# CityU-AIM-Group/SCAN

Hardware: AMD Instinct MI355X
Metric: train images/sec (whole node), VGG16 C2F 1024x2048 (higher is better)
Workload: dtype f32 (fp32 storage, fp32 multiply, fp32 accumulate -- the reference's arithmetic; the convolutions run it on the bf16 matrix cores as bf16x6: every fp32 operand cut into 3 bf16 pieces = all 24 significand bits, 6 bf16 MFMAs per product)

## Files before the change

### include/scan_hip.h

```cpp
#ifndef SCAN_HIP_H
#define SCAN_HIP_H

#include <stdint.h>

#ifdef __cplusplus
extern "C" {
#endif

#define SCAN_MAX_LEVELS 5

typedef struct {
  int32_t n_levels;
  int32_t n_images;
  int32_t h[SCAN_MAX_LEVELS];
  int32_t w[SCAN_MAX_LEVELS];
  int64_t row_off[SCAN_MAX_LEVELS + 1];
} scan_pyramid_t;

const char* scan_last_error(void);
int scan_abi_version(void);

#define SCAN_TUNE_UNKNOWN (-2147483647 - 1)
int scan_tune(const char* key, int value);
int scan_tune_get(const char* key);
// ... 377 lines not shown
int scan_gconv3x3_to1_dgrad(const float* dy, int32_t Ns, const scan_pyramid_t* d, int32_t G, int32_t Cg, const float* w,
                            const float* mask, float* dx, void* stream);
int scan_gconv3x3_to1_wgrad(const float* x, const float* dy, int32_t Ns, const scan_pyramid_t* d, int32_t G, int32_t Cg,
                            float* dw, int32_t accumulate, float* ws, void* stream);
int scan_gconv3x3_to1_backward(const float* x, const float* dy, int32_t Ns, const scan_pyramid_t* d, int32_t G, int32_t Cg,
                               const float* w, int32_t relu_mask, float* dx, float* dw, int32_t accumulate, float* ws,
                               void* stream);
int32_t scan_gconv3x3_to1_max_groups(void);
#define SCAN_GCONV_RUNS 1
#define SCAN_GCONV_LANE_MAPPED 2
#define SCAN_GCONV_BITS 4
#define SCAN_GCONV_ACT 8
int32_t scan_gconv3x3_to1_caps(int32_t G, int32_t Cg);
int scan_gconv3x3_to1_any_forward(const float* x, const scan_pyramid_t* d, int32_t G, int32_t Cg, const float* w,
                                  const float* bias, float* y, int32_t Ns, float* ws, void* stream);
int scan_gconv3x3_to1_any_dgrad(const float* dy, int32_t Ns, const scan_pyramid_t* d, int32_t G, int32_t Cg, const float* w,
                                const float* mask, float* dx, void* stream);
int scan_gconv3x3_to1_any_wgrad(const float* x, const float* dy, int32_t Ns, const scan_pyramid_t* d, int32_t G, int32_t Cg,
                                float* dw, int32_t accumulate, float* ws, void* stream);
int scan_gconv3x3_to1_any_backward(const float* x, const float* dy, int32_t Ns, const scan_pyramid_t* d, int32_t G, int32_t Cg,
                                   const float* w, int32_t relu_mask, float* dx, float* dw, int32_t accumulate, float* ws,
                                   void* stream);
int64_t scan_gconv3x3_to1_act_ws_floats(const scan_pyramid_t* d, int32_t G, int32_t Cg);
int scan_gconv3x3_to1_act_forward(const float* x, const scan_pyramid_t* d, int32_t G, int32_t Cg, const float* w,
                                  const float* bias, const float* a, int32_t lda, int32_t a_col0, const float* E, float* y,
                                  int32_t Ns, float* ws, void* stream);
int scan_gconv3x3_to1_act_backward(const float* x, const float* dy, int32_t Ns, const scan_pyramid_t* d, int32_t G, int32_t Cg,
                                   const float* w, const float* a, int32_t lda, int32_t a_col0, const float* E, float* dx,
                                   float* dw, int32_t accumulate, float* ws, void* stream);
int scan_gconv3x3_to1_act_grads(const float* dh, const scan_pyramid_t* d, int32_t G, int32_t Cg, const float* a, int32_t lda,
                                int32_t a_col0, const float* E, float* da, int32_t ldda, int32_t da_col0, float* dE,
                                int32_t accumulate, float* ws, void* stream);
int scan_gconv3x3_to1_act_backward_all(const float* x, const float* dy, int32_t Ns, const scan_pyramid_t* d, int32_t G,
                                       int32_t Cg, const float* w, const float* a, int32_t lda, int32_t a_col0, const float* E,
                                       float* dx, float* dw, float* da, int32_t ldda, int32_t da_col0, float* dE,
                                       int32_t accumulate, float* ws, void* stream);
int scan_gconv3x3_to1_forward_bits(const float* x, const scan_pyramid_t* d, int32_t G, int32_t Cg, const float* w,
                                   const float* bias, float* y, int32_t Ns, float* ws, uint32_t* relu_bits, void* stream);
int scan_gconv3x3_to1_backward_bits(const float* x, const float* dy, int32_t Ns, const scan_pyramid_t* d, int32_t G,
                                    int32_t Cg, const float* w, const uint32_t* relu_bits, float* dx, float* dw,
                                    int32_t accumulate, float* ws, void* stream);

int scan_resize_bilinear_u8(const uint8_t* src, int32_t H, int32_t W, uint8_t* tmp, uint8_t* dst, int32_t OH, int32_t OW,
                            const int32_t* xbounds, const int32_t* xcoef, int32_t kx, const int32_t* ybounds,
                            const int32_t* ycoef, int32_t ky, void* stream);

// ... 59 lines not shown
```

### scan_amd/_lib.py

```python
import ctypes
import os

_HERE = os.path.dirname(os.path.abspath(__file__))
LIB_PATH = os.environ.get("SCAN_HIP_LIB") or os.path.join(_HERE, "libscan_hip.so")

MAX_LEVELS = 5
TUNE_UNKNOWN = -2 ** 31
NMS_PANEL = 8192
NMS_MAX = 262144

c_i32, c_i64, c_f32, c_vp = ctypes.c_int32, ctypes.c_int64, ctypes.c_float, ctypes.c_void_p


class PyramidDesc(ctypes.Structure):
    _fields_ = [("n_levels", c_i32), ("n_images", c_i32), ("h", c_i32 * MAX_LEVELS), ("w", c_i32 * MAX_LEVELS),
                ("row_off", c_i64 * (MAX_LEVELS + 1))]


_PD = ctypes.POINTER(PyramidDesc)


class SgdSegment(ctypes.Structure):
    _fields_ = [("p", c_vp), ("g", c_vp), ("buf", c_vp), ("n", c_i64), ("lr", c_f32), ("wd", c_f32),
                ("first_step", c_i32), ("reserved", c_i32)]
# ... 178 lines not shown
    "scan_cka_unstack_grads": (ctypes.c_int, [ctypes.POINTER(CkaBranch), c_i32, c_i32, c_i32, c_i64, c_i64, c_i64, c_i64,
                                              c_i64, c_i32, c_i32, c_vp, c_vp, c_vp, c_vp, c_i32, c_vp]),
    "scan_gconv3x3_to1_ws_floats": (c_i64, [_PD, c_i32, c_i32]),
    "scan_gconv3x3_to1_max_groups": (c_i32, []),
    "scan_gconv3x3_to1_caps": (c_i32, [c_i32, c_i32]),
    "scan_gconv3x3_to1_any_forward": (ctypes.c_int, [c_vp, _PD, c_i32, c_i32, c_vp, c_vp, c_vp, c_i32, c_vp, c_vp]),
    "scan_gconv3x3_to1_any_dgrad": (ctypes.c_int, [c_vp, c_i32, _PD, c_i32, c_i32, c_vp, c_vp, c_vp, c_vp]),
    "scan_gconv3x3_to1_any_wgrad": (ctypes.c_int, [c_vp, c_vp, c_i32, _PD, c_i32, c_i32, c_vp, c_i32, c_vp, c_vp]),
    "scan_gconv3x3_to1_any_backward": (ctypes.c_int, [c_vp, c_vp, c_i32, _PD, c_i32, c_i32, c_vp, c_i32, c_vp, c_vp, c_i32,
                                                      c_vp, c_vp]),
    "scan_gconv3x3_to1_forward": (ctypes.c_int, [c_vp, _PD, c_i32, c_i32, c_vp, c_vp, c_vp, c_i32, c_vp, c_vp]),
    "scan_gconv3x3_to1_dgrad": (ctypes.c_int, [c_vp, c_i32, _PD, c_i32, c_i32, c_vp, c_vp, c_vp, c_vp]),
    "scan_gconv3x3_to1_wgrad": (ctypes.c_int, [c_vp, c_vp, c_i32, _PD, c_i32, c_i32, c_vp, c_i32, c_vp, c_vp]),
    "scan_gconv3x3_to1_backward": (ctypes.c_int, [c_vp, c_vp, c_i32, _PD, c_i32, c_i32, c_vp, c_i32, c_vp, c_vp, c_i32, c_vp,
                                                  c_vp]),
    "scan_gconv3x3_to1_forward_bits": (ctypes.c_int, [c_vp, _PD, c_i32, c_i32, c_vp, c_vp, c_vp, c_i32, c_vp, c_vp, c_vp]),
    "scan_gconv3x3_to1_backward_bits": (ctypes.c_int, [c_vp, c_vp, c_i32, _PD, c_i32, c_i32, c_vp, c_vp, c_vp, c_vp, c_i32,
                                                       c_vp, c_vp]),
    "scan_cka_stack_weights_split": (ctypes.c_int, [ctypes.POINTER(CkaBranch), c_i32, c_i32, c_i32, c_i64, c_i64, c_i64, c_i64,
                                                    c_i64, c_i32, c_vp, c_vp, c_vp, c_vp, c_vp, c_vp]),
    "scan_cka_unstack_grads_split": (ctypes.c_int, [ctypes.POINTER(CkaBranch), c_i32, c_i32, c_i32, c_i64, c_i64, c_i64, c_i64,
                                                    c_i64, c_i32, c_vp, c_vp, c_vp, c_vp, c_vp, c_i32, c_vp]),
    "scan_gconv3x3_to1_act_ws_floats": (c_i64, [_PD, c_i32, c_i32]),
    "scan_gconv3x3_to1_act_forward": (ctypes.c_int, [c_vp, _PD, c_i32, c_i32, c_vp, c_vp, c_vp, c_i32, c_i32, c_vp, c_vp, c_i32,
                                                     c_vp, c_vp]),
    "scan_gconv3x3_to1_act_backward": (ctypes.c_int, [c_vp, c_vp, c_i32, _PD, c_i32, c_i32, c_vp, c_vp, c_i32, c_i32, c_vp, c_vp,
                                                      c_vp, c_i32, c_vp, c_vp]),
    "scan_gconv3x3_to1_act_backward_all": (ctypes.c_int, [c_vp, c_vp, c_i32, _PD, c_i32, c_i32, c_vp, c_vp, c_i32, c_i32, c_vp,
                                                          c_vp, c_vp, c_vp, c_i32, c_i32, c_vp, c_i32, c_vp, c_vp]),
    "scan_gconv3x3_to1_act_grads": (ctypes.c_int, [c_vp, _PD, c_i32, c_i32, c_vp, c_i32, c_i32, c_vp, c_vp, c_i32, c_i32, c_vp,
                                                   c_i32, c_vp, c_vp]),
    "scan_resize_bilinear_u8": (ctypes.c_int, [c_vp, c_i32, c_i32, c_vp, c_vp, c_i32, c_i32, c_vp, c_vp, c_i32, c_vp, c_vp,
                                               c_i32, c_vp]),
    "scan_sigmoid_focal_loss_ordered_ws_floats": (c_i64, [c_i64, c_i32]),
    "scan_sigmoid_focal_loss_forward_ordered": (ctypes.c_int, [c_vp, c_vp, c_i64, c_i32, c_f32, c_f32, c_vp, c_vp, c_vp, c_vp]),
    "scan_iou_loss_ordered_ws_floats": (c_i64, [c_i64]),
    "scan_iou_loss_forward_ordered": (ctypes.c_int, [c_vp, c_vp, c_vp, c_i64, c_vp, c_vp, c_vp]),
    "scan_bce_logits_ordered_ws_floats": (c_i64, [c_i64]),
    "scan_bce_logits_forward_ordered": (ctypes.c_int, [c_vp, c_vp, c_f32, c_vp, c_i64, c_i64, c_vp, c_vp, c_vp]),
    "scan_cka_bce_ordered_ws_floats": (c_i64, [c_i64, c_i32]),
    "scan_cka_bce_forward_ordered": (ctypes.c_int, [c_vp, c_vp, c_i64, c_i32, c_f32, c_vp, c_vp, c_vp]),
    "scan_cka_bce_forward_loss_ordered": (ctypes.c_int, [c_vp, c_vp, c_i64, c_i32, c_f32, c_vp, c_vp, c_vp]),
    "scan_softmax_focal_ordered_ws_floats": (c_i64, [c_i64]),
    "scan_softmax_focal_forward_ordered": (ctypes.c_int, [c_vp, c_vp, c_i64, c_i32, c_f32, c_vp, c_vp, c_vp]),
    "scan_groupnorm_ordered_ws_floats": (c_i64, [_PD, c_i32, c_i32]),
    "scan_groupnorm_stats_ordered": (ctypes.c_int, [c_vp, _PD, c_i32, c_i32, c_f32, c_vp, c_vp, c_vp]),
# ... 85 lines not shown
```

### scan_amd/csrc/capi.cpp

```cpp
#include <stdarg.h>
#include <stdio.h>
#include <string.h>

#include "../../include/scan_hip.h"
#include "conv_launch.h"

static thread_local char g_err[512] = "";

extern "C" void scan_set_error(const char* fmt, ...) {
  va_list ap;
  va_start(ap, fmt);
  vsnprintf(g_err, sizeof(g_err), fmt, ap);
  va_end(ap);
}

extern "C" const char* scan_last_error(void) { return g_err; }
extern "C" int scan_abi_version(void) { return 1; }

int g_scan_deterministic = 0;

struct Knob {
  const char* key;
  int* slot;
  int dflt;
};
static Knob* knob_table(int* count) {
  static Knob knobs[] = {
      {"conv_bn256", &g_scan_conv_bn256, 0},   {"conv_v2", &g_scan_conv_v2, 0},         {"conv_wg1024", &g_scan_conv_wg1024, 0},
      {"conv_w8", &g_scan_conv_w8, 0},         {"conv_tpb3", &g_scan_conv_tpb3, 0},     {"conv_bn64_th16", &g_scan_conv_bn64_th16, 0},
      {"conv_glds", &g_scan_conv_glds, 0},     {"wgrad_v6", &g_scan_wgrad_v6, 0},       {"wgrad_prio", &g_scan_wgrad_prio, 0},
      {"wgrad_tile", &g_scan_wgrad_tile, 0},   {"wgrad_wgs", &g_scan_wgrad_wgs, 0},     {"gconv_mfma", &g_scan_gconv_mfma, 0},
      {"dbscan_bf16x3", &g_scan_dbscan_bf16x3, 0}, {"reduce_blocks", &g_scan_reduce_blocks, 0}, {"conv1x1", &g_scan_conv1x1, 0},
      {"conv_wino", &g_scan_conv_wino, 0},     {"wgrad_wino", &g_scan_wgrad_wino, 0},   {"wino_tpb", &g_scan_wino_tpb, 0},
      {"deterministic", &g_scan_deterministic, 0}, {"dynconv_generic", &g_scan_dynconv_generic, 0},
  };
  static bool init = false;
  if (!init) {
    for (auto& k : knobs) k.dflt = *k.slot;
    init = true;
  }
  *count = (int)(sizeof(knobs) / sizeof(knobs[0]));
  return knobs;
}
static Knob* find_knob(const char* key) {
  int n = 0;
  Knob* t = knob_table(&n);
  if (key == nullptr) return nullptr;
  for (int i = 0; i < n; ++i)
    if (strcmp(key, t[i].key) == 0) return &t[i];
  return nullptr;
}

extern "C" int scan_tune(const char* key, int value) {
  Knob* k = find_knob(key);
  if (k == nullptr) return SCAN_TUNE_UNKNOWN;
  const int old = *k->slot;
  *k->slot = value;
// ... 19 lines not shown
```

### scan_amd/csrc/conv_launch.h

```cpp
#pragma once
#include <hip/hip_runtime_api.h>
#include <stdint.h>

#include "../../include/scan_hip.h"

extern int g_scan_conv_v2;
extern int g_scan_conv_bn256, g_scan_conv_wg1024, g_scan_conv_w8, g_scan_conv_tpb3;
extern int g_scan_conv_glds, g_scan_conv_bn64_th16, g_scan_conv1x1;
extern int g_scan_conv_wino, g_scan_wino_tpb;
extern int g_scan_wgrad_v6, g_scan_wgrad_prio, g_scan_wgrad_tile, g_scan_wgrad_wgs, g_scan_wgrad_wino;
extern int g_scan_gconv_mfma;
extern int g_scan_dynconv_generic;
extern int g_scan_dbscan_bf16x3;
extern int g_scan_reduce_blocks;

struct ConvArgs {
  const float* x;
  const scan_pyramid_t* od;
  const scan_pyramid_t* sd;
  int32_t Cs;
  const __bf16* w[3];
  int32_t Csw;
  const float* bias;
  const float* mask;
  float* y;
  int32_t Nout, Ns, relu, map;
  hipStream_t st;
  double* gn_ws;
};

struct ConvInst {
  int id;
  void (*launch)(const ConvArgs&);
};
// ... 17 lines not shown
```

### scan_amd/csrc/gconv.hip

```cpp
#include "common.h"

#define GC_G 128

template <int CTRL, int ROW_MASK>
__device__ __forceinline__ float dpp_add(float v) {
  const int r = __builtin_amdgcn_update_dpp(0, __builtin_bit_cast(int, v), CTRL, ROW_MASK, 0xF, false);
  return v + __builtin_bit_cast(float, r);
}
__device__ __forceinline__ float half_wave_sum_hi(float v) {
  v = dpp_add<0xB1, 0xF>(v);
  v = dpp_add<0x4E, 0xF>(v);
  v = dpp_add<0x141, 0xF>(v);
  v = dpp_add<0x140, 0xF>(v);
  v = dpp_add<0x142, 0xA>(v);
  return v;
}

__device__ __forceinline__ int64_t neighbour_row(const scan_pyramid_t& d, int64_t m, const RowCoord& rc, int oy, int ox) {
  const int y = rc.y + oy, x = rc.x + ox;
  if (y < 0 || y >= d.h[rc.lvl] || x < 0 || x >= d.w[rc.lvl]) return -1;
  return m + (int64_t)oy * d.w[rc.lvl] + ox;
}

__device__ __forceinline__ float4 zero4() { return make_float4(0.f, 0.f, 0.f, 0.f); }
// ... 34 lines not shown
template <int SIGN>
__device__ __forceinline__ void tap_values(const scan_pyramid_t& d, int64_t q, const RowCoord& rc,
                                           const float* __restrict__ src, int ld, int g, bool uniform, float (&v)[9]) {
  if (uniform) {
    const int g0 = 2 * (int)(threadIdx.x >> 6);
    const int l = threadIdx.x & 63;
    const int tl = l % 9, gl = l / 9;
    const int64_t pl = l < 18 ? neighbour_row(d, q, rc, SIGN * (tl / 3 - 1), SIGN * (tl % 3 - 1)) : -1;
    const float val = pl >= 0 ? src[pl * ld + g0 + gl] : 0.f;
    const int vb = __builtin_bit_cast(int, val);
    const bool hi = (l & 32) != 0;
#pragma unroll
    for (int t = 0; t < 9; ++t) {
      const float lo_v = __builtin_bit_cast(float, __builtin_amdgcn_readlane(vb, t));
      const float hi_v = __builtin_bit_cast(float, __builtin_amdgcn_readlane(vb, 9 + t));
      v[t] = hi ? hi_v : lo_v;
    }
  } else {
#pragma unroll
    for (int t = 0; t < 9; ++t) {
      const int64_t p = neighbour_row(d, q, rc, SIGN * (t / 3 - 1), SIGN * (t % 3 - 1));
      v[t] = p >= 0 ? src[p * ld + g] : 0.f;
    }
  }
}

struct LaneMap {
  int g, l32, coff;
  int64_t first, stride, step;
  bool uniform;
};

__device__ __forceinline__ LaneMap slot_lanes(int GC, int un, bool runs) {
  const int quads = GC >> 2;
  const int slots = 256 / quads;
  const int cq = threadIdx.x % quads, slot = threadIdx.x / quads;
  LaneMap lm;
  lm.g = cq >> 5, lm.l32 = cq & 31, lm.coff = 4 * cq;
  lm.first = runs ? (int64_t)blockIdx.x * un * slots + slot : (int64_t)blockIdx.x * slots + slot;
  lm.stride = runs ? (int64_t)slots : (int64_t)gridDim.x * slots;
  lm.step = (int64_t)gridDim.x * un * slots;
  lm.uniform = slots == 1;
  return lm;
}

__device__ __forceinline__ int half_wave_id() { return blockIdx.x * 8 + (threadIdx.x >> 5); }
// ... 332 lines not shown
  const int t = i / GC, c = i - t * GC;
  return DST == GC_DST_DW ? ((int64_t)(c / GC_G) * 9 + t) * GC + c : ((int64_t)(c / GC_G) * 9 + t) * GC_G + c % GC_G;
}

template <GconvDst DST>
__global__ __launch_bounds__(256) void gconv_reduce_kernel(const float* __restrict__ partial, int parts, int GC,
                                                           float* __restrict__ out, int accumulate) {
  const int i = blockIdx.x * blockDim.x + threadIdx.x;
  if (i >= 9 * GC) return;
  float s = 0.f;
  for (int b = 0; b < parts; ++b) s += partial[(int64_t)b * 9 * GC + i];
  float* dst = out + gconv_dst_index<DST>(i, GC);
  *dst = accumulate ? *dst + s : s;
}


__device__ __forceinline__ float4 act_hidden(float4 h, const float4 (&ev)[9], const float (&av)[9]) {
#pragma unroll
  for (int t = 0; t < 9; ++t) fma4(h, av[t], ev[t]);
  return relu_mask4(h, h);
}

#define GC_UNROLL_A 2
#define GC_PICK_UNI(G, kernel, ...) ((G) == 8 ? kernel<true, ##__VA_ARGS__> : kernel<false, ##__VA_ARGS__>)

template <bool UNI>
__global__ __launch_bounds__(256) void gconv_taps_act_kernel(const float* __restrict__ x, scan_pyramid_t d, int G, int GC,
                                                             const float* __restrict__ w, const float* __restrict__ a,
                                                             int lda, const float* __restrict__ E, float* __restrict__ T) {
  const int64_t M = d.row_off[d.n_levels];
  const int quads = GC >> 2, slots = 256 / quads;
  const int cq = threadIdx.x % quads, slot = threadIdx.x / quads;
  const int g = cq >> 5, l32 = cq & 31;
  float4 wv[9], ev[9];
#pragma unroll
  for (int t = 0; t < 9; ++t) {
    wv[t] = *reinterpret_cast<const float4*>(w + ((int64_t)g * 9 + t) * GC + 4 * cq);
    ev[t] = *reinterpret_cast<const float4*>(E + ((int64_t)g * 9 + t) * GC_G + 4 * l32);
  }
  const int64_t stride = (int64_t)gridDim.x * slots;
  for (int64_t q0 = (int64_t)blockIdx.x * slots + slot; q0 < M; q0 += GC_UNROLL_F * stride) {
    float4 h[GC_UNROLL_F];
#pragma unroll
    for (int u = 0; u < GC_UNROLL_F; ++u) {
      const int64_t q = q0 + u * stride;
      h[u] = q < M ? *reinterpret_cast<const float4*>(x + q * GC + 4 * cq) : zero4();
    }
#pragma unroll
    for (int u = 0; u < GC_UNROLL_F; ++u) {
      int64_t q = q0 + u * stride;
      if (UNI) q = uniform_row(q);
      if (q >= M) continue;
      float av[9];
      tap_values<1>(d, q, decode_row(d, q), a, lda, g, UNI, av);
      tap_store(T, q, G, g, l32, tap_sums(act_hidden(h[u], ev, av), wv, l32));
    }
  }
}

template <bool UNI, bool FUSE>
__global__ __launch_bounds__(256, (UNI && !FUSE) ? 3 : 2) void gconv_bwd_act_kernel(
    const float* __restrict__ x, const float* __restrict__ dy, int Ns, scan_pyramid_t d, int G, int GC,
    const float* __restrict__ w, const float* __restrict__ a, int lda, const float* __restrict__ E, float* __restrict__ dx,
    float* __restrict__ slab, float* __restrict__ T, float* __restrict__ slab_e) {
  __shared__ float red[9 * 1024];
  const int64_t M = d.row_off[d.n_levels];
  const int quads = GC >> 2, slots = 256 / quads;
  const int cq = threadIdx.x % quads, slot = threadIdx.x / quads;
  const int g = cq >> 5, l32 = cq & 31;
  float4 wv[9], ev[9], acc[9], acc_e[9];
#pragma unroll
  for (int t = 0; t < 9; ++t) {
    wv[t] = *reinterpret_cast<const float4*>(w + ((int64_t)g * 9 + t) * GC + 4 * cq);
    ev[t] = *reinterpret_cast<const float4*>(E + ((int64_t)g * 9 + t) * GC_G + 4 * l32);
    acc[t] = zero4();
    if (FUSE) acc_e[t] = zero4();
  }
  for (int64_t q0 = (int64_t)blockIdx.x * GC_UNROLL_A * slots + slot; q0 < M;
       q0 += (int64_t)gridDim.x * GC_UNROLL_A * slots) {
    float4 h[GC_UNROLL_A];
#pragma unroll
    for (int u = 0; u < GC_UNROLL_A; ++u) {
      const int64_t q = q0 + u * slots;
      h[u] = q < M ? *reinterpret_cast<const float4*>(x + q * GC + 4 * cq) : zero4();
    }
#pragma unroll
    for (int u = 0; u < GC_UNROLL_A; ++u) {
      int64_t q = q0 + u * slots;
      if (UNI) q = uniform_row(q);
      if (q >= M) continue;
      const RowCoord rc = decode_row(d, q);
      float av[9], gy[9];
      tap_values<1>(d, q, rc, a, lda, g, UNI, av);
      const float4 hv = act_hidden(h[u], ev, av);
      tap_values<-1>(d, q, rc, dy, Ns, g, UNI, gy);
      float4 o = zero4();
#pragma unroll
      for (int t = 0; t < 9; ++t) {
        fma4(acc[t], gy[t], hv);
        fma4(o, gy[t], wv[t]);
      }
      o = relu_mask4(hv, o);
      *reinterpret_cast<float4*>(dx + q * GC + 4 * cq) = o;
      if (FUSE) {
        float mine = 0.f;
#pragma unroll
        for (int t = 0; t < 9; ++t) {
          fma4(acc_e[t], av[t], o);
          const float s = half_wave_sum_hi(dot4(o, ev[8 - t]));
          if (l32 == 16 + t) mine = s;
        }
        tap_store(T, q, G, g, l32, mine);
      }
    }
  }
  slab_store(acc, red, slab, GC);
  if (FUSE) {
    __syncthreads();
    slab_store(acc_e, red, slab_e, GC);
  }
}

template <bool UNI>
__global__ __launch_bounds__(256) void gconv_act_grads_kernel(const float* __restrict__ dh, scan_pyramid_t d, int G, int GC,
                                                              const float* __restrict__ a, int lda,
                                                              const float* __restrict__ E, float* __restrict__ T,
                                                              float* __restrict__ slab) {
  __shared__ float red[9 * 1024];
  const int64_t M = d.row_off[d.n_levels];
  const int quads = GC >> 2, slots = 256 / quads;
  const int cq = threadIdx.x % quads, slot = threadIdx.x / quads;
  const int g = cq >> 5, l32 = cq & 31;
  float4 ev[9], acc[9];
#pragma unroll
  for (int t = 0; t < 9; ++t) {
    ev[t] = *reinterpret_cast<const float4*>(E + ((int64_t)g * 9 + t) * GC_G + 4 * l32);
    acc[t] = zero4();
  }
  for (int64_t q0 = (int64_t)blockIdx.x * GC_UNROLL_A * slots + slot; q0 < M;
       q0 += (int64_t)gridDim.x * GC_UNROLL_A * slots) {
    float4 h[GC_UNROLL_A];
#pragma unroll
    for (int u = 0; u < GC_UNROLL_A; ++u) {
      const int64_t q = q0 + u * slots;
      h[u] = q < M ? *reinterpret_cast<const float4*>(dh + q * GC + 4 * cq) : zero4();
    }
#pragma unroll
    for (int u = 0; u < GC_UNROLL_A; ++u) {
      int64_t q = q0 + u * slots;
      if (UNI) q = uniform_row(q);
      if (q >= M) continue;
      float av[9];
      tap_values<1>(d, q, decode_row(d, q), a, lda, g, UNI, av);
      float mine = 0.f;
#pragma unroll
      for (int t = 0; t < 9; ++t) {
        fma4(acc[t], av[t], h[u]);
        const float s = half_wave_sum_hi(dot4(h[u], ev[8 - t]));
        if (l32 == 16 + t) mine = s;
      }
      tap_store(T, q, G, g, l32, mine);
    }
  }
  slab_store(acc, red, slab, GC);
}

#define GC_MAX_BLOCKS 1024
#define GC_PARTS 32
#define GC_GMAX 31

static bool gconv_lane_mapped(int G) { return G == 1 || G == 2 || G == 4 || G == 8; }

static int gconv_check(const scan_pyramid_t* d, int G, int Cg, const char* who, bool any_g = false) {
  SCAN_CHECK_ARG(d && d->n_levels >= 1 && d->n_levels <= SCAN_MAX_LEVELS, "%s: bad pyramid", who);
  SCAN_CHECK_ARG(Cg == GC_G, "%s: only 128 channels per group are built (got %d)", who, Cg);
  if (any_g) {
    SCAN_CHECK_ARG(G >= 1 && G <= GC_GMAX, "%s: G=%d out of 1..%d", who, G, GC_GMAX);
    return 0;
  }
  SCAN_CHECK_ARG(gconv_lane_mapped(G), "%s: G=%d must be 1, 2, 4 or 8", who, G);
  return 0;
}

int g_scan_gconv_mfma = 0;

enum GconvFamily { GC_GENERIC, GC_FMA, GC_MFMA };
static GconvFamily gconv_family(int G, bool bits) {
  if (!gconv_lane_mapped(G)) return GC_GENERIC;
  return (g_scan_gconv_mfma || bits) ? GC_MFMA : GC_FMA;
}

extern "C" int32_t scan_gconv3x3_to1_max_groups(void) { return GC_GMAX; }

extern "C" int32_t scan_gconv3x3_to1_caps(int32_t G, int32_t Cg) {
  if (G < 1 || G > GC_GMAX || Cg != GC_G) return 0;
  const GconvFamily f = gconv_family(G, false);
  return SCAN_GCONV_RUNS | (f == GC_GENERIC ? 0 : SCAN_GCONV_LANE_MAPPED) | (f == GC_MFMA ? SCAN_GCONV_BITS : 0) |
         (f == GC_FMA ? SCAN_GCONV_ACT : 0);
}

struct GconvWs {
  int64_t slab, slab_e, total;
};
static GconvWs gconv_ws_layout(int64_t M, int G, int Cg, bool act) {
  const int64_t taps = M * G * 9, slab = (int64_t)(GC_MAX_BLOCKS + GC_PARTS) * 9 * G * Cg;
  if (act) return {taps, taps + slab, taps + 2 * slab};
  return {0, -1, taps > slab ? taps : slab};
}

extern "C" int64_t scan_gconv3x3_to1_ws_floats(const scan_pyramid_t* d, int32_t G, int32_t Cg) {
  return d ? gconv_ws_layout(d->row_off[d->n_levels], G, Cg, false).total : -1;
}

extern "C" int64_t scan_gconv3x3_to1_act_ws_floats(const scan_pyramid_t* d, int32_t G, int32_t Cg) {
  return d ? gconv_ws_layout(d->row_off[d->n_levels], G, Cg, true).total : -1;
}

static int gconv_generic_strides(int64_t M, int per, int max_j) {
  int64_t j = ((M + per - 1) / per + 7) / 8 * 8;
  if (j < 8) j = 8;
  if (j > max_j) j = max_j;
  return (int)j;
}

static int gconv_slab_blocks(int64_t M) {
  int64_t rpb = (M + GC_MAX_BLOCKS - 1) / GC_MAX_BLOCKS;
  if (rpb < 16) rpb = 16;
  return (int)((M + rpb - 1) / rpb);
}

static int gconv_wave_grid(int64_t M, int G) {
  int64_t tasks = ((M + 15) / 16) * G;
  int64_t blocks = (tasks + 3) / 4;
  if (blocks > 2048) blocks = 2048;
  if (blocks < 2) blocks = 2;
  return (int)((blocks + 1) / 2 * 2);
}

static int gconv_gather(const float* T, const scan_pyramid_t* d, int G, const float* bias, float* y, int ldy, int col0,
                        hipStream_t st) {
  const int64_t M = d->row_off[d->n_levels];
  hipLaunchKernelGGL(gconv_gather_kernel, dim3(grid_for(M * ldy, 256)), dim3(256), 0, st, T, *d, G, bias, y, ldy, col0);
  SCAN_LAUNCH_CHECK("gconv_gather");
  return 0;
}

template <GconvDst DST>
static int gconv_slab_to(float* slab, int blocks, int GC, float* out, int accumulate, hipStream_t st) {
  const int n = 9 * GC, per = (blocks + GC_PARTS - 1) / GC_PARTS, parts = (blocks + per - 1) / per;
  float* partial = slab + (int64_t)GC_MAX_BLOCKS * n;
  hipLaunchKernelGGL(gconv_slab_partial_kernel, dim3((n + 255) / 256, parts), dim3(256), 0, st, slab, blocks, n, per, partial);
// ... 1 lines not shown
  hipLaunchKernelGGL(gconv_reduce_kernel<DST>, dim3((n + 255) / 256), dim3(256), 0, st, partial, parts, GC, out, accumulate);
  SCAN_LAUNCH_CHECK(DST == GC_DST_DE ? "gconv_act_reduce" : "gconv_wgrad_reduce");
  return 0;
}

static int gconv_forward(const float* x, const scan_pyramid_t* d, int G, int Cg, const float* w, const float* bias, float* y,
                         int Ns, float* ws, uint32_t* relu_bits, hipStream_t st, bool any_g = false) {
  if (gconv_check(d, G, Cg, "gconv3x3_to1_forward", any_g)) return -1;
  SCAN_CHECK_ARG(x && w && y && ws && Ns >= G, "gconv3x3_to1_forward: bad arguments (Ns=%d)", Ns);
  const int64_t M = d->row_off[d->n_levels];
  if (M == 0) return 0;
  const int GC = G * Cg;
  switch (gconv_family(G, relu_bits != nullptr)) {
    case GC_GENERIC:
      SCAN_CHECK_ARG(relu_bits == nullptr, "gconv3x3_to1_forward_bits: G=%d must be 1, 2, 4 or 8", G);
      hipLaunchKernelGGL(gconv_taps_generic_kernel, dim3(gconv_generic_strides(M, GC_UNROLL_F, 2048) / 8 * G), dim3(256), 0,
                         st, x, M, G, GC, w, ws);
      SCAN_LAUNCH_CHECK("gconv_taps_generic");
      break;
    case GC_MFMA:
      hipLaunchKernelGGL(gconv_taps_mfma_kernel, dim3(gconv_wave_grid(M, G)), dim3(256), 0, st, x, M, G, GC, w, ws, relu_bits);
      SCAN_LAUNCH_CHECK("gconv_taps");
      break;
    case GC_FMA: {
      const int slots = 256 / (GC / 4);
      hipLaunchKernelGGL(gconv_taps_kernel, dim3(grid_for((M + slots - 1) / slots, 1)), dim3(256), 0, st, x, M, G, GC, w, ws);
      SCAN_LAUNCH_CHECK("gconv_taps");
    }
  }
  return gconv_gather(ws, d, G, bias, y, Ns, 0, st);
}

template <bool DO_DX, bool DO_DW>
static void gconv_bwd_launch(bool generic, int grid, hipStream_t st, const float* x, const float* dy, int Ns,
                             const scan_pyramid_t* d, int G, int GC, const float* w, int relu_mask, float* dx, float* slab) {
  hipLaunchKernelGGL((generic ? gconv_bwd_generic_kernel<DO_DX, DO_DW> : gconv_bwd_kernel<DO_DX, DO_DW>), dim3(grid), dim3(256),
                     0, st, x, dy, Ns, *d, G, GC, w, relu_mask, dx, slab);
}

static int gconv_backward(const float* x, const float* dy, int Ns, const scan_pyramid_t* d, int G, int Cg, const float* w,
                          int relu_mask, const uint32_t* relu_bits, float* dx, float* dw, int accumulate, float* ws,
                          hipStream_t st, const char* who, bool any_g = false) {
  if (gconv_check(d, G, Cg, who, any_g)) return -1;
  SCAN_CHECK_ARG(dy && Ns >= G && (dx || dw), "%s: bad arguments (Ns=%d)", who, Ns);
  SCAN_CHECK_ARG(!dx || w, "%s: the data gradient needs the weights", who);
  SCAN_CHECK_ARG(!dw || (x && ws), "%s: the weight gradient needs x and a workspace", who);
  SCAN_CHECK_ARG(!(dx && relu_mask && !relu_bits) || x, "%s: the ReLU mask needs x or its bit mask", who);
  const int64_t M = d->row_off[d->n_levels];
  if (M == 0) return 0;
  const int GC = G * Cg;
  const GconvFamily family = gconv_family(G, relu_bits != nullptr);
// ... 77 lines not shown
extern "C" int scan_gconv3x3_to1_any_wgrad(const float* x, const float* dy, int32_t Ns, const scan_pyramid_t* d, int32_t G,
                                           int32_t Cg, float* dw, int32_t accumulate, float* ws, void* stream) {
  SCAN_CHECK_ARG(dw, "gconv3x3_to1_any_wgrad: null output");
  return gconv_backward(x, dy, Ns, d, G, Cg, nullptr, 0, nullptr, nullptr, dw, accumulate, ws, as_stream(stream),
                        "gconv3x3_to1_any_wgrad", true);
}

extern "C" int scan_gconv3x3_to1_any_backward(const float* x, const float* dy, int32_t Ns, const scan_pyramid_t* d, int32_t G,
                                              int32_t Cg, const float* w, int32_t relu_mask, float* dx, float* dw,
                                              int32_t accumulate, float* ws, void* stream) {
  SCAN_CHECK_ARG(x && dx && dw, "gconv3x3_to1_any_backward: null pointer");
  return gconv_backward(x, dy, Ns, d, G, Cg, w, relu_mask, nullptr, dx, dw, accumulate, ws, as_stream(stream),
                        "gconv3x3_to1_any_backward", true);
}

static int gconv_act_check(const scan_pyramid_t* d, int G, int Cg, const float* a, int lda, int a_col0, const float* E,
                           const char* who) {
  if (gconv_check(d, G, Cg, who)) return -1;
  SCAN_CHECK_ARG(a && E && a_col0 >= 0 && lda >= a_col0 + G, "%s: bad act map (lda=%d, first column %d, G=%d)", who, lda,
                 a_col0, G);
  return 0;
}

extern "C" int scan_gconv3x3_to1_act_forward(const float* x, const scan_pyramid_t* d, int32_t G, int32_t Cg, const float* w,
                                             const float* bias, const float* a, int32_t lda, int32_t a_col0, const float* E,
                                             float* y, int32_t Ns, float* ws, void* stream) {
  if (gconv_act_check(d, G, Cg, a, lda, a_col0, E, "gconv3x3_to1_act_forward")) return -1;
  SCAN_CHECK_ARG(x && w && y && ws && Ns >= G, "gconv3x3_to1_act_forward: bad arguments (Ns=%d)", Ns);
  const int64_t M = d->row_off[d->n_levels];
  if (M == 0) return 0;
  const int GC = G * Cg, slots = 256 / (GC / 4);
  hipStream_t st = as_stream(stream);
  hipLaunchKernelGGL(GC_PICK_UNI(G, gconv_taps_act_kernel), dim3(grid_for((M + slots - 1) / slots, 1)), dim3(256), 0, st, x, *d,
                     G, GC, w, a + a_col0, lda, E, ws);
  SCAN_LAUNCH_CHECK("gconv_taps_act");
  return gconv_gather(ws, d, G, bias, y, Ns, 0, st);
}

extern "C" int scan_gconv3x3_to1_act_backward(const float* x, const float* dy, int32_t Ns, const scan_pyramid_t* d, int32_t G,
                                              int32_t Cg, const float* w, const float* a, int32_t lda, int32_t a_col0,
                                              const float* E, float* dx, float* dw, int32_t accumulate, float* ws,
                                              void* stream) {
  if (gconv_act_check(d, G, Cg, a, lda, a_col0, E, "gconv3x3_to1_act_backward")) return -1;
  SCAN_CHECK_ARG(x && dy && w && dx && dw && ws && Ns >= G, "gconv3x3_to1_act_backward: bad arguments (Ns=%d)", Ns);
  const int64_t M = d->row_off[d->n_levels];
  if (M == 0) return 0;
  const int GC = G * Cg, blocks = gconv_slab_blocks(M);
  hipStream_t st = as_stream(stream);
  float* slab = ws + gconv_ws_layout(M, G, Cg, true).slab;
  hipLaunchKernelGGL(GC_PICK_UNI(G, gconv_bwd_act_kernel, false), dim3(blocks), dim3(256), 0, st, x, dy, Ns, *d, G, GC, w,
                     a + a_col0, lda, E, dx, slab, (float*)nullptr, (float*)nullptr);
  SCAN_LAUNCH_CHECK("gconv_bwd_act");
  return gconv_slab_to<GC_DST_DW>(slab, blocks, GC, dw, accumulate, st);
}

extern "C" int scan_gconv3x3_to1_act_grads(const float* dh, const scan_pyramid_t* d, int32_t G, int32_t Cg, const float* a,
                                           int32_t lda, int32_t a_col0, const float* E, float* da, int32_t ldda,
                                           int32_t da_col0, float* dE, int32_t accumulate, float* ws, void* stream) {
  if (gconv_act_check(d, G, Cg, a, lda, a_col0, E, "gconv3x3_to1_act_grads")) return -1;
  SCAN_CHECK_ARG(dh && da && dE && ws && da_col0 >= 0 && ldda >= da_col0 + G,
                 "gconv3x3_to1_act_grads: bad arguments (ldda=%d, first column %d)", ldda, da_col0);
  const int64_t M = d->row_off[d->n_levels];
  if (M == 0) return 0;
  const int GC = G * Cg, blocks = gconv_slab_blocks(M);
  hipStream_t st = as_stream(stream);
  float* slab = ws + gconv_ws_layout(M, G, Cg, true).slab;
  hipLaunchKernelGGL(GC_PICK_UNI(G, gconv_act_grads_kernel), dim3(blocks), dim3(256), 0, st, dh, *d, G, GC, a + a_col0, lda, E,
                     ws, slab);
  SCAN_LAUNCH_CHECK("gconv_act_grads");
  if (int rc = gconv_gather(ws, d, G, nullptr, da, ldda, da_col0, st)) return rc;
  return gconv_slab_to<GC_DST_DE>(slab, blocks, GC, dE, accumulate, st);
}

extern "C" int scan_gconv3x3_to1_act_backward_all(const float* x, const float* dy, int32_t Ns, const scan_pyramid_t* d,
                                                  int32_t G, int32_t Cg, const float* w, const float* a, int32_t lda,
                                                  int32_t a_col0, const float* E, float* dx, float* dw, float* da, int32_t ldda,
                                                  int32_t da_col0, float* dE, int32_t accumulate, float* ws, void* stream) {
  if (gconv_act_check(d, G, Cg, a, lda, a_col0, E, "gconv3x3_to1_act_backward_all")) return -1;
  SCAN_CHECK_ARG(x && dy && w && dx && dw && ws && Ns >= G, "gconv3x3_to1_act_backward_all: bad arguments (Ns=%d)", Ns);
  SCAN_CHECK_ARG(da && dE && da_col0 >= 0 && ldda >= da_col0 + G,
                 "gconv3x3_to1_act_backward_all: bad arguments (ldda=%d, first column %d)", ldda, da_col0);
  const int64_t M = d->row_off[d->n_levels];
  if (M == 0) return 0;
  const int GC = G * Cg, blocks = gconv_slab_blocks(M);
  hipStream_t st = as_stream(stream);
  const GconvWs L = gconv_ws_layout(M, G, Cg, true);
  hipLaunchKernelGGL(GC_PICK_UNI(G, gconv_bwd_act_kernel, true), dim3(blocks), dim3(256), 0, st, x, dy, Ns, *d, G, GC, w,
                     a + a_col0, lda, E, dx, ws + L.slab, ws, ws + L.slab_e);
  SCAN_LAUNCH_CHECK("gconv_bwd_act");
  if (int rc = gconv_gather(ws, d, G, nullptr, da, ldda, da_col0, st)) return rc;
  if (int rc = gconv_slab_to<GC_DST_DW>(ws + L.slab, blocks, GC, dw, accumulate, st)) return rc;
  return gconv_slab_to<GC_DST_DE>(ws + L.slab_e, blocks, GC, dE, accumulate, st);
}
```

Measured before the change: 25.76.

## Software-pipeline gconv act kernels with lane-spread neighbour tap fetches

```diff
diff --git a/include/scan_hip.h b/include/scan_hip.h
--- a/include/scan_hip.h
+++ b/include/scan_hip.h
@@ -423,6 +423,7 @@
                                    const float* w, int32_t relu_mask, float* dx, float* dw, int32_t accumulate, float* ws,
                                    void* stream);
 int64_t scan_gconv3x3_to1_act_ws_floats(const scan_pyramid_t* d, int32_t G, int32_t Cg);
+int32_t scan_gconv3x3_to1_act_blocks(const scan_pyramid_t* d, int32_t G, int32_t Cg, int32_t backward);
 int scan_gconv3x3_to1_act_forward(const float* x, const scan_pyramid_t* d, int32_t G, int32_t Cg, const float* w,
                                   const float* bias, const float* a, int32_t lda, int32_t a_col0, const float* E, float* y,
                                   int32_t Ns, float* ws, void* stream);
diff --git a/scan_amd/_lib.py b/scan_amd/_lib.py
--- a/scan_amd/_lib.py
+++ b/scan_amd/_lib.py
@@ -224,6 +224,7 @@
     "scan_cka_unstack_grads_split": (ctypes.c_int, [ctypes.POINTER(CkaBranch), c_i32, c_i32, c_i32, c_i64, c_i64, c_i64, c_i64,
                                                     c_i64, c_i32, c_vp, c_vp, c_vp, c_vp, c_vp, c_i32, c_vp]),
     "scan_gconv3x3_to1_act_ws_floats": (c_i64, [_PD, c_i32, c_i32]),
+    "scan_gconv3x3_to1_act_blocks": (c_i32, [_PD, c_i32, c_i32, c_i32]),
     "scan_gconv3x3_to1_act_forward": (ctypes.c_int, [c_vp, _PD, c_i32, c_i32, c_vp, c_vp, c_vp, c_i32, c_i32, c_vp, c_vp, c_i32,
                                                      c_vp, c_vp]),
     "scan_gconv3x3_to1_act_backward": (ctypes.c_int, [c_vp, c_vp, c_i32, _PD, c_i32, c_i32, c_vp, c_vp, c_i32, c_i32, c_vp, c_vp,
diff --git a/scan_amd/csrc/capi.cpp b/scan_amd/csrc/capi.cpp
--- a/scan_amd/csrc/capi.cpp
+++ b/scan_amd/csrc/capi.cpp
@@ -33,6 +33,7 @@
       {"dbscan_bf16x3", &g_scan_dbscan_bf16x3, 0}, {"reduce_blocks", &g_scan_reduce_blocks, 0}, {"conv1x1", &g_scan_conv1x1, 0},
       {"conv_wino", &g_scan_conv_wino, 0},     {"wgrad_wino", &g_scan_wgrad_wino, 0},   {"wino_tpb", &g_scan_wino_tpb, 0},
       {"deterministic", &g_scan_deterministic, 0}, {"dynconv_generic", &g_scan_dynconv_generic, 0},
+      {"gconv_act_pipe", &g_scan_gconv_act_pipe, 0},
   };
   static bool init = false;
   if (!init) {
diff --git a/scan_amd/csrc/conv_launch.h b/scan_amd/csrc/conv_launch.h
--- a/scan_amd/csrc/conv_launch.h
+++ b/scan_amd/csrc/conv_launch.h
@@ -9,7 +9,7 @@
 extern int g_scan_conv_glds, g_scan_conv_bn64_th16, g_scan_conv1x1;
 extern int g_scan_conv_wino, g_scan_wino_tpb;
 extern int g_scan_wgrad_v6, g_scan_wgrad_prio, g_scan_wgrad_tile, g_scan_wgrad_wgs, g_scan_wgrad_wino;
-extern int g_scan_gconv_mfma;
+extern int g_scan_gconv_mfma, g_scan_gconv_act_pipe;
 extern int g_scan_dynconv_generic;
 extern int g_scan_dbscan_bf16x3;
 extern int g_scan_reduce_blocks;
diff --git a/scan_amd/csrc/gconv.hip b/scan_amd/csrc/gconv.hip
--- a/scan_amd/csrc/gconv.hip
+++ b/scan_amd/csrc/gconv.hip
@@ -80,6 +80,32 @@
       const int64_t p = neighbour_row(d, q, rc, SIGN * (t / 3 - 1), SIGN * (t % 3 - 1));
       v[t] = p >= 0 ? src[p * ld + g] : 0.f;
     }
+  }
+}
+
+template <int SIGN, bool PAIR>
+__device__ __forceinline__ float2 tap_fetch(const scan_pyramid_t& d, bool live, int64_t q, const RowCoord& rc,
+                                            const float* __restrict__ src, int ld, int col) {
+  const int l = threadIdx.x & 63, t = l % 9;
+  const int64_t pl = (live && l < (PAIR ? 9 : 18)) ? neighbour_row(d, q, rc, SIGN * (t / 3 - 1), SIGN * (t % 3 - 1)) : -1;
+  const float* at = src + (pl >= 0 ? pl : q) * ld + col;
+  float2 v = make_float2(0.f, 0.f);
+  if (PAIR)
+    __builtin_memcpy(&v, at, sizeof(v));
+  else
+    v.x = *at;
+  return pl >= 0 ? v : make_float2(0.f, 0.f);
+}
+
+template <bool PAIR>
+__device__ __forceinline__ void tap_spread(const float2& fetched, float (&v)[9]) {
+  const int lo = __builtin_bit_cast(int, fetched.x), up = __builtin_bit_cast(int, PAIR ? fetched.y : fetched.x);
+  const bool hi = (threadIdx.x & 32) != 0;
+#pragma unroll
+  for (int t = 0; t < 9; ++t) {
+    const float lo_v = __builtin_bit_cast(float, __builtin_amdgcn_readlane(lo, t));
+    const float hi_v = __builtin_bit_cast(float, __builtin_amdgcn_readlane(up, PAIR ? t : 9 + t));
+    v[t] = hi ? hi_v : lo_v;
   }
 }
 
@@ -458,9 +484,40 @@
 }
 
 #define GC_UNROLL_A 2
-#define GC_PICK_UNI(G, kernel, ...) ((G) == 8 ? kernel<true, ##__VA_ARGS__> : kernel<false, ##__VA_ARGS__>)
-
+#define GC_PICK_ACT(G, kernel, ...)                                                                               \
+  ((G) == 8 ? (g_scan_gconv_act_pipe == 1 ? kernel<true, ##__VA_ARGS__, true> : kernel<true, ##__VA_ARGS__, false>) \
+            : (g_scan_gconv_act_pipe == 1 ? kernel<false, ##__VA_ARGS__, true> : kernel<false, ##__VA_ARGS__, false>))
+
+struct ActRow {
+  float4 h;
+  float2 ta, td;
+};
+struct FetchLane {
+  int g, dslot;
+};
 template <bool UNI>
+__device__ __forceinline__ FetchLane act_fetch_lane(int quads) {
+  const int l = threadIdx.x & 63;
+  const int ft = (threadIdx.x & ~63) + ((!UNI && l >= 9) ? 32 : 0);
+  return {(ft % quads) >> 5, ft / quads - (int)threadIdx.x / quads};
+}
+template <bool UNI, bool DY>
+__device__ __forceinline__ ActRow act_row_fetch(const float* __restrict__ x, const scan_pyramid_t& d, int64_t M, int64_t q,
+                                                int GC, int cq, const FetchLane& fl, const float* __restrict__ a, int lda,
+                                                const float* __restrict__ dy, int Ns) {
+  if (UNI) q = uniform_row(q);
+  ActRow r;
+  r.h = *reinterpret_cast<const float4*>(x + (q < M ? q : M - 1) * GC + 4 * cq);
+  int64_t qf = UNI ? q : q + fl.dslot;
+  const bool live = qf < M;
+  qf = live ? qf : M - 1;
+  const RowCoord rc = decode_row(d, qf);
+  r.ta = tap_fetch<1, UNI>(d, live, qf, rc, a, lda, fl.g);
+  r.td = DY ? tap_fetch<-1, UNI>(d, live, qf, rc, dy, Ns, fl.g) : make_float2(0.f, 0.f);
+  return r;
+}
+
+template <bool UNI, bool PIPE>
 __global__ __launch_bounds__(256) void gconv_taps_act_kernel(const float* __restrict__ x, scan_pyramid_t d, int G, int GC,
                                                              const float* __restrict__ w, const float* __restrict__ a,
                                                              int lda, const float* __restrict__ E, float* __restrict__ T) {
@@ -475,6 +532,31 @@
     ev[t] = *reinterpret_cast<const float4*>(E + ((int64_t)g * 9 + t) * GC_G + 4 * l32);
   }
   const int64_t stride = (int64_t)gridDim.x * slots;
+  if (PIPE) {
+    ActRow row[GC_UNROLL_F], next[GC_UNROLL_F];
+    const FetchLane fl = act_fetch_lane<UNI>(quads);
+    const int64_t first = (int64_t)blockIdx.x * slots + slot;
+#pragma unroll
+    for (int u = 0; u < GC_UNROLL_F; ++u)
+      row[u] = act_row_fetch<UNI, false>(x, d, M, first + u * stride, GC, cq, fl, a, lda, nullptr, 0);
+    for (int64_t q0 = first; q0 < M; q0 += GC_UNROLL_F * stride) {
+#pragma unroll
+      for (int u = 0; u < GC_UNROLL_F; ++u)
+        next[u] = act_row_fetch<UNI, false>(x, d, M, q0 + (u + GC_UNROLL_F) * stride, GC, cq, fl, a, lda, nullptr, 0);
+#pragma unroll
+      for (int u = 0; u < GC_UNROLL_F; ++u) {
+        int64_t q = q0 + u * stride;
+        if (UNI) q = uniform_row(q);
+        if (q >= M) continue;
+        float av[9];
+        tap_spread<UNI>(row[u].ta, av);
+        tap_store(T, q, G, g, l32, tap_sums(act_hidden(row[u].h, ev, av), wv, l32));
+      }
+#pragma unroll
+      for (int u = 0; u < GC_UNROLL_F; ++u) row[u] = next[u];
+    }
+    return;
+  }
   for (int64_t q0 = (int64_t)blockIdx.x * slots + slot; q0 < M; q0 += GC_UNROLL_F * stride) {
     float4 h[GC_UNROLL_F];
 #pragma unroll
@@ -494,8 +576,33 @@
   }
 }
 
-template <bool UNI, bool FUSE>
-__global__ __launch_bounds__(256, (UNI && !FUSE) ? 3 : 2) void gconv_bwd_act_kernel(
+template <bool FUSE>
+__device__ __forceinline__ void bwd_act_row(const float4& hv, const float (&av)[9], const float (&gy)[9], const float4 (&wv)[9],
+                                            const float4 (&ev)[9], float4 (&acc)[9], float4 (&acc_e)[9],
+                                            float* __restrict__ dx, float* __restrict__ T, int64_t q, int G, int GC, int cq) {
+  const int g = cq >> 5, l32 = cq & 31;
+  float4 o = zero4();
+#pragma unroll
+  for (int t = 0; t < 9; ++t) {
+    fma4(acc[t], gy[t], hv);
+    fma4(o, gy[t], wv[t]);
+  }
+  o = relu_mask4(hv, o);
+  *reinterpret_cast<float4*>(dx + q * GC + 4 * cq) = o;
+  if (FUSE) {
+    float mine = 0.f;
+#pragma unroll
+    for (int t = 0; t < 9; ++t) {
+      fma4(acc_e[t], av[t], o);
+      const float s = half_wave_sum_hi(dot4(o, ev[8 - t]));
+      if (l32 == 16 + t) mine = s;
+    }
+    tap_store(T, q, G, g, l32, mine);
+  }
+}
+
+template <bool UNI, bool FUSE, bool PIPE>
+__global__ __launch_bounds__(256, (UNI && !FUSE && !PIPE) ? 3 : 2) void gconv_bwd_act_kernel(
     const float* __restrict__ x, const float* __restrict__ dy, int Ns, scan_pyramid_t d, int G, int GC,
     const float* __restrict__ w, const float* __restrict__ a, int lda, const float* __restrict__ E, float* __restrict__ dx,
     float* __restrict__ slab, float* __restrict__ T, float* __restrict__ slab_e) {
@@ -503,50 +610,59 @@
   const int64_t M = d.row_off[d.n_levels];
   const int quads = GC >> 2, slots = 256 / quads;
   const int cq = threadIdx.x % quads, slot = threadIdx.x / quads;
-  const int g = cq >> 5, l32 = cq & 31;
+  const int g = cq >> 5;
   float4 wv[9], ev[9], acc[9], acc_e[9];
 #pragma unroll
   for (int t = 0; t < 9; ++t) {
     wv[t] = *reinterpret_cast<const float4*>(w + ((int64_t)g * 9 + t) * GC + 4 * cq);
-    ev[t] = *reinterpret_cast<const float4*>(E + ((int64_t)g * 9 + t) * GC_G + 4 * l32);
+    ev[t] = *reinterpret_cast<const float4*>(E + ((int64_t)g * 9 + t) * GC_G + 4 * (cq & 31));
     acc[t] = zero4();
     if (FUSE) acc_e[t] = zero4();
   }
-  for (int64_t q0 = (int64_t)blockIdx.x * GC_UNROLL_A * slots + slot; q0 < M;
-       q0 += (int64_t)gridDim.x * GC_UNROLL_A * slots) {
+  const int64_t first = (int64_t)blockIdx.x * GC_UNROLL_A * slots + slot, step = (int64_t)gridDim.x * GC_UNROLL_A * slots;
+  if (PIPE) {
+    ActRow row[GC_UNROLL_A], next[GC_UNROLL_A];
+    const FetchLane fl = act_fetch_lane<UNI>(quads);
+#pragma unroll
+    for (int u = 0; u < GC_UNROLL_A; ++u)
+      row[u] = act_row_fetch<UNI, true>(x, d, M, first + u * slots, GC, cq, fl, a, lda, dy, Ns);
+    for (int64_t q0 = first; q0 < M; q0 += step) {
+#pragma unroll
+      for (int u = 0; u < GC_UNROLL_A; ++u)
+        next[u] = act_row_fetch<UNI, true>(x, d, M, q0 + step + u * slots, GC, cq, fl, a, lda, dy, Ns);
+#pragma unroll
+      for (int u = 0; u < GC_UNROLL_A; ++u) {
+        int64_t q = q0 + u * slots;
+        if (UNI) q = uniform_row(q);
+        if (q >= M) continue;
+        float av[9], gy[9];
+        tap_spread<UNI>(row[u].ta, av);
+        const float4 hv = act_hidden(row[u].h, ev, av);
+        tap_spread<UNI>(row[u].td, gy);
+        bwd_act_row<FUSE>(hv, av, gy, wv, ev, acc, acc_e, dx, T, q, G, GC, cq);
+      }
+#pragma unroll
+      for (int u = 0; u < GC_UNROLL_A; ++u) row[u] = next[u];
+    }
+  } else {
     float4 h[GC_UNROLL_A];
-#pragma unroll
-    for (int u = 0; u < GC_UNROLL_A; ++u) {
-      const int64_t q = q0 + u * slots;
-      h[u] = q < M ? *reinterpret_cast<const float4*>(x + q * GC + 4 * cq) : zero4();
-    }
-#pragma unroll
-    for (int u = 0; u < GC_UNROLL_A; ++u) {
-      int64_t q = q0 + u * slots;
-      if (UNI) q = uniform_row(q);
-      if (q >= M) continue;
-      const RowCoord rc = decode_row(d, q);
-      float av[9], gy[9];
-      tap_values<1>(d, q, rc, a, lda, g, UNI, av);
-      const float4 hv = act_hidden(h[u], ev, av);
-      tap_values<-1>(d, q, rc, dy, Ns, g, UNI, gy);
-      float4 o = zero4();
-#pragma unroll
-      for (int t = 0; t < 9; ++t) {
-        fma4(acc[t], gy[t], hv);
-        fma4(o, gy[t], wv[t]);
-      }
-      o = relu_mask4(hv, o);
-      *reinterpret_cast<float4*>(dx + q * GC + 4 * cq) = o;
-      if (FUSE) {
-        float mine = 0.f;
-#pragma unroll
-        for (int t = 0; t < 9; ++t) {
-          fma4(acc_e[t], av[t], o);
-          const float s = half_wave_sum_hi(dot4(o, ev[8 - t]));
-          if (l32 == 16 + t) mine = s;
-        }
-        tap_store(T, q, G, g, l32, mine);
+    for (int64_t q0 = first; q0 < M; q0 += step) {
+#pragma unroll
+      for (int u = 0; u < GC_UNROLL_A; ++u) {
+        const int64_t q = q0 + u * slots;
+        h[u] = q < M ? *reinterpret_cast<const float4*>(x + q * GC + 4 * cq) : zero4();
+      }
+#pragma unroll
+      for (int u = 0; u < GC_UNROLL_A; ++u) {
+        int64_t q = q0 + u * slots;
+        if (UNI) q = uniform_row(q);
+        if (q >= M) continue;
+        const RowCoord rc = decode_row(d, q);
+        float av[9], gy[9];
+        tap_values<1>(d, q, rc, a, lda, g, UNI, av);
+        const float4 hv = act_hidden(h[u], ev, av);
+        tap_values<-1>(d, q, rc, dy, Ns, g, UNI, gy);
+        bwd_act_row<FUSE>(hv, av, gy, wv, ev, acc, acc_e, dx, T, q, G, GC, cq);
       }
     }
   }
@@ -557,7 +673,20 @@
   }
 }
 
-template <bool UNI>
+__device__ __forceinline__ void act_grads_row(const float4& h, const float (&av)[9], const float4 (&ev)[9], float4 (&acc)[9],
+                                              float* __restrict__ T, int64_t q, int G, int cq) {
+  const int g = cq >> 5, l32 = cq & 31;
+  float mine = 0.f;
+#pragma unroll
+  for (int t = 0; t < 9; ++t) {
+    fma4(acc[t], av[t], h);
+    const float s = half_wave_sum_hi(dot4(h, ev[8 - t]));
+    if (l32 == 16 + t) mine = s;
+  }
+  tap_store(T, q, G, g, l32, mine);
+}
+
+template <bool UNI, bool PIPE>
 __global__ __launch_bounds__(256) void gconv_act_grads_kernel(const float* __restrict__ dh, scan_pyramid_t d, int G, int GC,
                                                               const float* __restrict__ a, int lda,
                                                               const float* __restrict__ E, float* __restrict__ T,
@@ -566,36 +695,53 @@
   const int64_t M = d.row_off[d.n_levels];
   const int quads = GC >> 2, slots = 256 / quads;
   const int cq = threadIdx.x % quads, slot = threadIdx.x / quads;
-  const int g = cq >> 5, l32 = cq & 31;
+  const int g = cq >> 5;
   float4 ev[9], acc[9];
 #pragma unroll
   for (int t = 0; t < 9; ++t) {
-    ev[t] = *reinterpret_cast<const float4*>(E + ((int64_t)g * 9 + t) * GC_G + 4 * l32);
+    ev[t] = *reinterpret_cast<const float4*>(E + ((int64_t)g * 9 + t) * GC_G + 4 * (cq & 31));
     acc[t] = zero4();
   }
-  for (int64_t q0 = (int64_t)blockIdx.x * GC_UNROLL_A * slots + slot; q0 < M;
-       q0 += (int64_t)gridDim.x * GC_UNROLL_A * slots) {
+  const int64_t first = (int64_t)blockIdx.x * GC_UNROLL_A * slots + slot, step = (int64_t)gridDim.x * GC_UNROLL_A * slots;
+  if (PIPE) {
+    ActRow row[GC_UNROLL_A], next[GC_UNROLL_A];
+    const FetchLane fl = act_fetch_lane<UNI>(quads);
+#pragma unroll
+    for (int u = 0; u < GC_UNROLL_A; ++u)
+      row[u] = act_row_fetch<UNI, false>(dh, d, M, first + u * slots, GC, cq, fl, a, lda, nullptr, 0);
+    for (int64_t q0 = first; q0 < M; q0 += step) {
+#pragma unroll
+      for (int u = 0; u < GC_UNROLL_A; ++u)
+        next[u] = act_row_fetch<UNI, false>(dh, d, M, q0 + step + u * slots, GC, cq, fl, a, lda, nullptr, 0);
+#pragma unroll
+      for (int u = 0; u < GC_UNROLL_A; ++u) {
+        int64_t q = q0 + u * slots;
+        if (UNI) q = uniform_row(q);
+        if (q >= M) continue;
+        float av[9];
+        tap_spread<UNI>(row[u].ta, av);
+        act_grads_row(row[u].h, av, ev, acc, T, q, G, cq);
+      }
+#pragma unroll
+      for (int u = 0; u < GC_UNROLL_A; ++u) row[u] = next[u];
+    }
+  } else {
     float4 h[GC_UNROLL_A];
-#pragma unroll
-    for (int u = 0; u < GC_UNROLL_A; ++u) {
-      const int64_t q = q0 + u * slots;
-      h[u] = q < M ? *reinterpret_cast<const float4*>(dh + q * GC + 4 * cq) : zero4();
-    }
-#pragma unroll
-    for (int u = 0; u < GC_UNROLL_A; ++u) {
-      int64_t q = q0 + u * slots;
-      if (UNI) q = uniform_row(q);
-      if (q >= M) continue;
-      float av[9];
-      tap_values<1>(d, q, decode_row(d, q), a, lda, g, UNI, av);
-      float mine = 0.f;
-#pragma unroll
-      for (int t = 0; t < 9; ++t) {
-        fma4(acc[t], av[t], h[u]);
-        const float s = half_wave_sum_hi(dot4(h[u], ev[8 - t]));
-        if (l32 == 16 + t) mine = s;
-      }
-      tap_store(T, q, G, g, l32, mine);
+    for (int64_t q0 = first; q0 < M; q0 += step) {
+#pragma unroll
+      for (int u = 0; u < GC_UNROLL_A; ++u) {
+        const int64_t q = q0 + u * slots;
+        h[u] = q < M ? *reinterpret_cast<const float4*>(dh + q * GC + 4 * cq) : zero4();
+      }
+#pragma unroll
+      for (int u = 0; u < GC_UNROLL_A; ++u) {
+        int64_t q = q0 + u * slots;
+        if (UNI) q = uniform_row(q);
+        if (q >= M) continue;
+        float av[9];
+        tap_values<1>(d, q, decode_row(d, q), a, lda, g, UNI, av);
+        act_grads_row(h[u], av, ev, acc, T, q, G, cq);
+      }
     }
   }
   slab_store(acc, red, slab, GC);
@@ -619,6 +765,8 @@
 }
 
 int g_scan_gconv_mfma = 0;
+
+int g_scan_gconv_act_pipe = 1;
 
 enum GconvFamily { GC_GENERIC, GC_FMA, GC_MFMA };
 static GconvFamily gconv_family(int G, bool bits) {
@@ -663,6 +811,11 @@
   int64_t rpb = (M + GC_MAX_BLOCKS - 1) / GC_MAX_BLOCKS;
   if (rpb < 16) rpb = 16;
   return (int)((M + rpb - 1) / rpb);
+}
+
+static int gconv_taps_blocks(int64_t M, int GC) {
+  const int slots = 256 / (GC / 4);
+  return grid_for((M + slots - 1) / slots, 1);
 }
 
 static int gconv_wave_grid(int64_t M, int G) {
@@ -710,11 +863,9 @@
       hipLaunchKernelGGL(gconv_taps_mfma_kernel, dim3(gconv_wave_grid(M, G)), dim3(256), 0, st, x, M, G, GC, w, ws, relu_bits);
       SCAN_LAUNCH_CHECK("gconv_taps");
       break;
-    case GC_FMA: {
-      const int slots = 256 / (GC / 4);
-      hipLaunchKernelGGL(gconv_taps_kernel, dim3(grid_for((M + slots - 1) / slots, 1)), dim3(256), 0, st, x, M, G, GC, w, ws);
+    case GC_FMA:
+      hipLaunchKernelGGL(gconv_taps_kernel, dim3(gconv_taps_blocks(M, GC)), dim3(256), 0, st, x, M, G, GC, w, ws);
       SCAN_LAUNCH_CHECK("gconv_taps");
-    }
   }
   return gconv_gather(ws, d, G, bias, y, Ns, 0, st);
 }
@@ -838,6 +989,13 @@
   return 0;
 }
 
+extern "C" int32_t scan_gconv3x3_to1_act_blocks(const scan_pyramid_t* d, int32_t G, int32_t Cg, int32_t backward) {
+  if (gconv_check(d, G, Cg, "gconv3x3_to1_act_blocks")) return -1;
+  const int64_t M = d->row_off[d->n_levels];
+  if (M == 0) return 0;
+  return backward ? gconv_slab_blocks(M) : gconv_taps_blocks(M, G * Cg);
+}
+
 extern "C" int scan_gconv3x3_to1_act_forward(const float* x, const scan_pyramid_t* d, int32_t G, int32_t Cg, const float* w,
                                              const float* bias, const float* a, int32_t lda, int32_t a_col0, const float* E,
                                              float* y, int32_t Ns, float* ws, void* stream) {
@@ -845,10 +1003,10 @@
   SCAN_CHECK_ARG(x && w && y && ws && Ns >= G, "gconv3x3_to1_act_forward: bad arguments (Ns=%d)", Ns);
   const int64_t M = d->row_off[d->n_levels];
   if (M == 0) return 0;
-  const int GC = G * Cg, slots = 256 / (GC / 4);
+  const int GC = G * Cg;
   hipStream_t st = as_stream(stream);
-  hipLaunchKernelGGL(GC_PICK_UNI(G, gconv_taps_act_kernel), dim3(grid_for((M + slots - 1) / slots, 1)), dim3(256), 0, st, x, *d,
-                     G, GC, w, a + a_col0, lda, E, ws);
+  hipLaunchKernelGGL(GC_PICK_ACT(G, gconv_taps_act_kernel), dim3(gconv_taps_blocks(M, GC)), dim3(256), 0, st, x, *d, G, GC, w,
+                     a + a_col0, lda, E, ws);
   SCAN_LAUNCH_CHECK("gconv_taps_act");
   return gconv_gather(ws, d, G, bias, y, Ns, 0, st);
 }
@@ -864,7 +1022,7 @@
   const int GC = G * Cg, blocks = gconv_slab_blocks(M);
   hipStream_t st = as_stream(stream);
   float* slab = ws + gconv_ws_layout(M, G, Cg, true).slab;
-  hipLaunchKernelGGL(GC_PICK_UNI(G, gconv_bwd_act_kernel, false), dim3(blocks), dim3(256), 0, st, x, dy, Ns, *d, G, GC, w,
+  hipLaunchKernelGGL(GC_PICK_ACT(G, gconv_bwd_act_kernel, false), dim3(blocks), dim3(256), 0, st, x, dy, Ns, *d, G, GC, w,
                      a + a_col0, lda, E, dx, slab, (float*)nullptr, (float*)nullptr);
   SCAN_LAUNCH_CHECK("gconv_bwd_act");
   return gconv_slab_to<GC_DST_DW>(slab, blocks, GC, dw, accumulate, st);
@@ -881,7 +1039,7 @@
   const int GC = G * Cg, blocks = gconv_slab_blocks(M);
   hipStream_t st = as_stream(stream);
   float* slab = ws + gconv_ws_layout(M, G, Cg, true).slab;
-  hipLaunchKernelGGL(GC_PICK_UNI(G, gconv_act_grads_kernel), dim3(blocks), dim3(256), 0, st, dh, *d, G, GC, a + a_col0, lda, E,
+  hipLaunchKernelGGL(GC_PICK_ACT(G, gconv_act_grads_kernel), dim3(blocks), dim3(256), 0, st, dh, *d, G, GC, a + a_col0, lda, E,
                      ws, slab);
   SCAN_LAUNCH_CHECK("gconv_act_grads");
   if (int rc = gconv_gather(ws, d, G, nullptr, da, ldda, da_col0, st)) return rc;
@@ -901,7 +1059,7 @@
   const int GC = G * Cg, blocks = gconv_slab_blocks(M);
   hipStream_t st = as_stream(stream);
   const GconvWs L = gconv_ws_layout(M, G, Cg, true);
-  hipLaunchKernelGGL(GC_PICK_UNI(G, gconv_bwd_act_kernel, true), dim3(blocks), dim3(256), 0, st, x, dy, Ns, *d, G, GC, w,
+  hipLaunchKernelGGL(GC_PICK_ACT(G, gconv_bwd_act_kernel, true), dim3(blocks), dim3(256), 0, st, x, dy, Ns, *d, G, GC, w,
                      a + a_col0, lda, E, dx, ws + L.slab, ws, ws + L.slab_e);
   SCAN_LAUNCH_CHECK("gconv_bwd_act");
   if (int rc = gconv_gather(ws, d, G, nullptr, da, ldda, da_col0, st)) return rc;
```

New measurement: 25.75. Within noise of the previous version (-0.0%).
